# knights-lab/UTree

Measured on NVIDIA B200. Metric: reads/sec (150bp, L2-scale CTR, RC); k-mer lookups/sec in lookups_per_s, higher is better.
Workload: dtype u64

## Files before the change

### utree_b200/csrc/kernels.cu

```cuda
#include <cuda_runtime.h>
#include <stdint.h>
#include <stdio.h>
#include <stdlib.h>
#include <string.h>
#include "utb_internal.h"

#define SUFMASK 0xFFFFFFFFFFull
#define HIT_MISS 0xFFFFFFFFu
#define HIT_NOWIN 0xFFFFFFFEu

#define CK(call)                                                                 \
    do {                                                                         \
        cudaError_t e_ = (call);                                                 \
        if (e_ != cudaSuccess) {                                                 \
            utb_set_error("CUDA error %s at %s:%d (%s)", cudaGetErrorName(e_),   \
                          __FILE__, __LINE__, cudaGetErrorString(e_));           \
            return UTB_ERR_CUDA;                                                 \
        }                                                                        \
    } while (0)

struct DevDB {
    const uint32_t *binix32;
    const uint64_t *binix64;
    const uint8_t *recs;
// ... 354 lines not shown
    if ((uint32_t)p == db.quirk_bin) ++a;
    for (uint64_t i = a + gl; i < b; i += G) {
        const uint64_t word = (p << 40) | load_suffix(db.recs, i * db.sz);
        const uint64_t rc = revcomp_word(word);
        uint32_t *blk = sieve + 2ull * sv_index(db, sv_minimizer(word, rc), sv_block((uint32_t)(word >> 32), (uint32_t)(rc >> 32)));
        const uint2 m = sv_masks((uint32_t)(word >> 32), (uint32_t)word);
        atomicOr(blk + 0, m.x); atomicOr(blk + 1, m.y);
    }
}

#define COUNTER_SLOTS 1024
template <int NSTR, bool TABLE>
__global__ void __launch_bounds__(256, 6)
lookup_kernel(DevDB db, const uint64_t *__restrict__ pk, const uint32_t *__restrict__ bad,
              uint32_t n_pos, const uint32_t *__restrict__ n_groups_dev, uint32_t *__restrict__ hits, unsigned long long *__restrict__ counters) {
    if (n_groups_dev) n_pos = *n_groups_dev * 32u;
    const uint64_t slot = (uint64_t)blockIdx.x * blockDim.x + threadIdx.x;
    const uint32_t pos = (uint32_t)(NSTR == 2 ? slot >> 1 : slot);
    uint64_t w = 0;
    const bool valid = pos < n_pos && window_at(pk, bad, pos, w);
    uint32_t r = HIT_NOWIN, ns = 0;
    if (valid) {
        if (NSTR == 2 && (slot & 1)) w = revcomp_word(w);
        if (TABLE) r = kt_lookup(db, w, &ns);
        else {
            Probe q[1];
            probe_begin(db, w, q[0]);
            probe_run<1>(db, q);
            r = probe_end(db, q[0]);
        }
    }
    if (pos < n_pos) hits[slot] = r;
    const uint32_t nv = __popc(__ballot_sync(0xFFFFFFFFu, valid));
    const uint32_t nh = __popc(__ballot_sync(0xFFFFFFFFu, r < HIT_NOWIN));
    for (int o = 16; o; o >>= 1) ns += __shfl_xor_sync(0xFFFFFFFFu, ns, o);
    if ((threadIdx.x & 31u) == 0) {
        const uint32_t c = blockIdx.x & (COUNTER_SLOTS - 1);
        if (nv) atomicAdd(counters + c, (unsigned long long)nv);
        if (nh) atomicAdd(counters + COUNTER_SLOTS + c, (unsigned long long)nh);
        if (ns) atomicAdd(counters + 3 * COUNTER_SLOTS + c, (unsigned long long)ns);
    }
}

#define Q_CHUNK 128u
#define Q_INVALID 0xFFFFFFFFu
struct WarpQueue {
    uint64_t base;
    uint32_t used;
    bool have;
};
__device__ __forceinline__ void wq_init(WarpQueue &q) { q.base = 0; q.used = Q_CHUNK; q.have = false; }
__device__ __forceinline__ void wq_retire(const WarpQueue &q, uint32_t lane, uint32_t *__restrict__ q_slots) {
    if (q.have) for (uint32_t j = q.used + lane; j < Q_CHUNK; j += 32) q_slots[q.base + j] = Q_INVALID;
}
__device__ __forceinline__ void wq_reserve(WarpQueue &q, uint32_t c, uint32_t lane, uint32_t *__restrict__ q_slots,
                                           unsigned long long *__restrict__ q_count, uint64_t q_cap) {
    if (q.used + c <= Q_CHUNK) return;
    wq_retire(q, lane, q_slots);
    unsigned long long nb = 0;
    if (lane == 0) nb = atomicAdd(q_count, (unsigned long long)Q_CHUNK);
    q.base = __shfl_sync(0xFFFFFFFFu, nb, 0);
    q.used = 0;
    q.have = q.base + Q_CHUNK <= q_cap;
}
struct HitSink {
    uint32_t *hits;
    uint32_t *hitmap;
    const uint32_t *rid, *grp_off;
    uint32_t *cnt;
    uint32_t sh;
};
__device__ __forceinline__ void sink_put(const HitSink &k, uint32_t slot, uint32_t r) {
    if (k.cnt) {
        const uint32_t rd = __ldg(k.rid + (slot >> k.sh));
        k.hits[((uint64_t)__ldg(k.grp_off + rd) << k.sh) + atomicAdd(k.cnt + rd, 1u)] = r;
    } else { k.hits[slot] = r; atomicOr(k.hitmap + (slot >> 5), 1u << (slot & 31u)); }
}
__device__ __noinline__ uint32_t resolve_inline(const DevDB &db, uint64_t w, uint32_t slot, const HitSink &sink) {
    const uint32_t r = kt_lookup(db, w);
    if (r == HIT_MISS) return 0;
    sink_put(sink, slot, r);
    return 1;
}
template <int NSTR>
__device__ __forceinline__ uint32_t emit_survivors(const DevDB &db, WarpQueue &wq, uint32_t lane, bool passF, bool passR, uint64_t w, uint64_t rc,
                                                   uint32_t pos, uint64_t *__restrict__ q_words, uint32_t *__restrict__ q_slots,
                                                   unsigned long long *__restrict__ q_count, uint64_t q_cap, const HitSink &sink) {
    const uint32_t bF = __ballot_sync(0xFFFFFFFFu, passF);
    const uint32_t bR = NSTR == 2 ? __ballot_sync(0xFFFFFFFFu, passR) : 0u;
    const uint32_t cF = __popc(bF), c = cF + __popc(bR);
    uint32_t nh = 0;
    if (!c) return 0;
    wq_reserve(wq, c, lane, q_slots, q_count, q_cap);
    const uint32_t lt = (1u << lane) - 1u;
    if (wq.have) {
        const uint64_t at = wq.base + wq.used;
        if (passF) { const uint64_t i = at + __popc(bF & lt); q_words[i] = w; q_slots[i] = pos * NSTR; }
        if (passR) { const uint64_t i = at + cF + __popc(bR & lt); q_words[i] = rc; q_slots[i] = pos * NSTR + 1u; }
    } else {
        if (passF) nh += resolve_inline(db, w, pos * NSTR, sink);
        if (passR) nh += resolve_inline(db, rc, pos * NSTR + 1u, sink);
    }
    wq.used += c;
    return nh;
}

#define SV_DEAD 0xFFFFFFFFu
struct SvStep { uint32_t wh, wl, rh, rl, h, blk; };
struct SvWords { uint64_t hi, lo, rhi, rlo; uint32_t bh, bl; };
__device__ __forceinline__ void sv_step(const SvWords &g, bool upper, uint32_t r2, uint32_t lane, SvStep &s) {
    const uint32_t b0 = (uint32_t)(g.hi >> 32), b1 = (uint32_t)g.hi, b2 = (uint32_t)(g.lo >> 32), b3 = (uint32_t)g.lo;
    const uint32_t x0 = upper ? b1 : b0, x1 = upper ? b2 : b1, x2 = upper ? b3 : b2;
    s.wh = __funnelshift_l(x1, x0, r2); s.wl = __funnelshift_l(x2, x1, r2);
    const uint32_t a0 = (uint32_t)(g.rlo >> 32), a1 = (uint32_t)g.rlo, a2 = (uint32_t)(g.rhi >> 32), a3 = (uint32_t)g.rhi;
    const uint32_t z0 = upper ? a2 : a3, z1 = upper ? a1 : a2, z2 = upper ? a0 : a1;
    s.rl = __funnelshift_r(z0, z1, r2); s.rh = __funnelshift_r(z1, z2, r2);
    s.h = sv_mhash(s.wh, s.rl);
    s.blk = __funnelshift_r(g.bh, g.bl, lane) == 0u ? sv_block(s.wh, s.rh) : SV_DEAD;
}
template <int D, int SV_U>
__device__ __forceinline__ void sv_shifted(const uint32_t (&x)[SV_U + 1], uint32_t (&y)[SV_U + 1], uint32_t lane) {
    uint32_t rot[SV_U + 1];
#pragma unroll
    for (int u = 0; u <= SV_U; ++u) rot[u] = __shfl_sync(0xFFFFFFFFu, x[u], (lane + D) & 31u);
    const bool same = lane + D < 32u;
#pragma unroll
    for (int u = 0; u < SV_U; ++u) y[u] = same ? rot[u] : rot[u + 1];
    y[SV_U] = rot[SV_U];
}
__device__ __forceinline__ void sv_prefetch(const void *p) { asm volatile("prefetch.global.L1 [%0];" ::"l"(p)); }
template <int NSTR, int SV_U, int SV_MINB>
__global__ void __launch_bounds__(256, SV_MINB)
sieve_kernel(DevDB db, const uint64_t *__restrict__ pk, const uint32_t *__restrict__ bad, const uint64_t *__restrict__ pkr, uint32_t n_pos,
             const uint32_t *__restrict__ n_groups_dev, unsigned long long *__restrict__ counters,
             uint64_t *__restrict__ q_words, uint32_t *__restrict__ q_slots, unsigned long long *__restrict__ q_count,
             uint64_t q_cap, const HitSink sink) {
    if (n_groups_dev) n_pos = *n_groups_dev * 32u;
    const uint32_t lane = threadIdx.x & 31u;
    const bool upper = lane >= 16u;
    const uint32_t r2 = 2u * (lane & 15u);
    const uint32_t n_steps = n_pos >> 5;
    const uint32_t n_warps = gridDim.x * (blockDim.x >> 5), wid = blockIdx.x * (blockDim.x >> 5) + (threadIdx.x >> 5);
    uint32_t per = (n_steps + n_warps - 1) / n_warps;
    per = (per + SV_U - 1) / SV_U * SV_U;
    const uint64_t s0 = (uint64_t)wid * per;
    const uint32_t s1 = s0 + per < n_steps ? (uint32_t)(s0 + per) : n_steps;
    const uint2 *__restrict__ sieve = db.sieve;
    const uint32_t n_lines = db.sv_lines;
    WarpQueue wq;
    wq_init(wq);
    uint32_t nv = 0, nh = 0;
    if (s0 < s1) {
        SvStep st[SV_U + 1];
        SvWords g;
        g.hi = __ldg(pk + s0); g.rhi = __ldg(pkr + s0); g.bh = __ldg(bad + s0);
        g.lo = __ldg(pk + s0 + 1); g.rlo = __ldg(pkr + s0 + 1); g.bl = __ldg(bad + s0 + 1);
        sv_step(g, upper, r2, lane, st[0]);
        for (uint32_t s = (uint32_t)s0; s < s1; s += SV_U) {
            {
                const uint32_t pf = s + 32u < n_steps ? s + 32u : n_steps;
                sv_prefetch(pk + pf); sv_prefetch(pkr + pf); sv_prefetch(bad + pf);
            }
#pragma unroll
            for (int u = 1; u <= SV_U; ++u) {
                g.hi = g.lo; g.rhi = g.rlo; g.bh = g.bl;
                g.lo = __ldg(pk + s + u + 1); g.rlo = __ldg(pkr + s + u + 1); g.bl = __ldg(bad + s + u + 1);
                sv_step(g, upper, r2, lane, st[u]);
            }
            uint32_t x[SV_U + 1], y1[SV_U + 1], y2[SV_U + 1];
#pragma unroll
            for (int u = 0; u <= SV_U; ++u) x[u] = st[u].h;
            sv_shifted<1, SV_U>(x, y1, lane); sv_shifted<2, SV_U>(x, y2, lane);
#pragma unroll
            for (int u = 0; u <= SV_U; ++u) x[u] = __vimin3_u32(x[u], y1[u], y2[u]);
            sv_shifted<3, SV_U>(x, y1, lane); sv_shifted<6, SV_U>(x, y2, lane);
#pragma unroll
            for (int u = 0; u <= SV_U; ++u) x[u] = __vimin3_u32(x[u], y1[u], y2[u]);
            sv_shifted<8, SV_U>(x, y1, lane);
#pragma unroll
            for (int u = 0; u < SV_U; ++u) x[u] = x[u] < y1[u] ? x[u] : y1[u];
            uint2 v[SV_U];
#pragma unroll
            for (int u = 0; u < SV_U; ++u) {
                v[u] = make_uint2(0, 0);
                if (st[u].blk != SV_DEAD) v[u] = __ldg(sieve + ((sv_line(x[u], n_lines) << 4) | st[u].blk));
            }
#pragma unroll
            for (int u = 0; u < SV_U; ++u) {
                const bool live = st[u].blk != SV_DEAD;
                if (__any_sync(0xFFFFFFFFu, live)) {
                    const bool tF = sv_test(v[u], st[u].wh, st[u].wl), tR = NSTR == 2 && sv_test(v[u], st[u].rh, st[u].rl);
                    nh += emit_survivors<NSTR>(db, wq, lane, live & tF, live & tR, ((uint64_t)st[u].wh << 32) | st[u].wl, ((uint64_t)st[u].rh << 32) | st[u].rl,
                                               (s + u) * 32u + lane, q_words, q_slots, q_count, q_cap, sink);
                    nv += live ? NSTR : 0;
                }
            }
            st[0] = st[SV_U];
        }
    }
    wq_retire(wq, lane, q_slots);
    for (int o = 16; o; o >>= 1) { nv += __shfl_xor_sync(0xFFFFFFFFu, nv, o); nh += __shfl_xor_sync(0xFFFFFFFFu, nh, o); }
    if (lane == 0) {
        const uint32_t cs = (blockIdx.x * 8 + (threadIdx.x >> 5)) & (COUNTER_SLOTS - 1);
        if (nv) atomicAdd(counters + cs, (unsigned long long)nv);
        if (nh) atomicAdd(counters + COUNTER_SLOTS + cs, (unsigned long long)nh);
    }
}

template <bool LISTS>
__global__ void __launch_bounds__(256, 6)
queue_lookup_kernel(DevDB db, const uint64_t *__restrict__ q_words, const uint32_t *__restrict__ q_slots,
                    const unsigned long long *__restrict__ q_count, uint64_t q_cap,
                    const HitSink sink, unsigned long long *__restrict__ counters) {
    const uint64_t n = *q_count < q_cap ? *q_count : q_cap;
    const uint64_t stride = (uint64_t)gridDim.x * blockDim.x;
    const uint32_t lane = threadIdx.x & 31u;
    uint32_t nh = 0, nsect = 0;
    for (uint64_t i = (uint64_t)blockIdx.x * blockDim.x + threadIdx.x; i < n; i += stride) {
        const uint32_t slot = q_slots[i];
        uint32_t r = HIT_MISS;
        if (slot != Q_INVALID) {
            uint32_t sc;
            r = kt_lookup(db, q_words[i], &sc);
            nsect += sc;
        }
        const bool hit = r != HIT_MISS;
        nh += hit;
        if (!LISTS) {
            if (hit) { sink.hits[slot] = r; atomicOr(sink.hitmap + (slot >> 5), 1u << (slot & 31u)); }
            continue;
        }
        if (!__any_sync(0xFFFFFFFFu, hit)) continue;
        const uint32_t rd = hit ? __ldg(sink.rid + (slot >> sink.sh)) : 0xFFFFFFFFu;
        const uint32_t peers = __match_any_sync(0xFFFFFFFFu, rd);
        const uint32_t leader = (uint32_t)__ffs(peers) - 1u;
        uint32_t base = 0;
        if (hit && lane == leader) base = atomicAdd(sink.cnt + rd, (uint32_t)__popc(peers));
        base = __shfl_sync(0xFFFFFFFFu, base, leader);
        if (hit) sink.hits[((uint64_t)__ldg(sink.grp_off + rd) << sink.sh) + base + __popc(peers & ((1u << lane) - 1u))] = r;
    }
    for (int o = 16; o; o >>= 1) { nh += __shfl_xor_sync(0xFFFFFFFFu, nh, o); nsect += __shfl_xor_sync(0xFFFFFFFFu, nsect, o); }
    if (lane == 0) {
        const uint32_t c = blockIdx.x & (COUNTER_SLOTS - 1);
        if (nh) atomicAdd(counters + COUNTER_SLOTS + c, (unsigned long long)nh);
        if (nsect) atomicAdd(counters + 3 * COUNTER_SLOTS + c, (unsigned long long)nsect);
    }
}

template <bool TABLE>
__global__ void lookup_words_kernel(DevDB db, const uint64_t *__restrict__ words, uint64_t n, uint32_t *__restrict__ ix) {
    uint64_t i = (uint64_t)blockIdx.x * blockDim.x + threadIdx.x;
    if (i >= n) return;
    if (TABLE) {
        if (db.sieve && !sv_maybe(db, words[i])) { ix[i] = HIT_MISS; return; }
        ix[i] = kt_lookup(db, words[i]);
        return;
    }
    Probe q[1];
    probe_begin(db, words[i], q[0]);
    probe_run<1>(db, q);
    ix[i] = probe_end(db, q[0]);
}


__global__ void expand_windows_kernel(const uint64_t *__restrict__ pk, const uint32_t *__restrict__ bad, uint32_t n_pos,
                                      uint64_t *__restrict__ fwd, uint64_t *__restrict__ rc, uint8_t *__restrict__ valid) {
    uint32_t pos = blockIdx.x * blockDim.x + threadIdx.x;
    if (pos >= n_pos) return;
    uint64_t w;
    bool ok = window_at(pk, bad, pos, w);
    fwd[pos] = ok ? w : 0;
    rc[pos] = ok ? revcomp_word(w) : 0;
    valid[pos] = ok;
}

__device__ __forceinline__ uint32_t cutoff_of(uint32_t x) {
    uint32_t c = x - x / 4u;
    c += ((x >> 1) >= c);
    return c;
}

__device__ __forceinline__ unsigned long long nz_bytes(unsigned long long v) {
    return (((v & 0x7F7F7F7F7F7F7F7Full) + 0x7F7F7F7F7F7F7F7Full) | v) & 0x8080808080808080ull;
}
__device__ __forceinline__ uint32_t scan_token(const char *s1, const char *s2, uint32_t t, char &a, char &b) {
    uint32_t tb = t & ~7u;
    unsigned long long keep = ~0ull << (8u * (t & 7u));
    for (;;) {
        const unsigned long long x1 = *reinterpret_cast<const unsigned long long *>(s1 + tb);
        const unsigned long long x2 = *reinterpret_cast<const unsigned long long *>(s2 + tb);
        const unsigned long long stop = ((nz_bytes(x1) & nz_bytes(x1 ^ 0x3B3B3B3B3B3B3B3Bull)) ^ 0x8080808080808080ull | nz_bytes(x1 ^ x2)) & keep;
        if (stop) {
            const uint32_t k = ((uint32_t)__ffsll((long long)stop) - 1u) >> 3;
            a = (char)(x1 >> (8u * k)); b = (char)(x2 >> (8u * k));
            return tb + k;
        }
        tb += 8u; keep = ~0ull;
    }
}

__device__ void walk_warp(const DevDB &db, const uint32_t *T_lab, const uint32_t *T_cnt,
                          uint32_t uix, uint32_t n, utb_result *out) {
    const uint32_t lane = threadIdx.x & 31u;
    const uint32_t EMPTY = 0xFFFFFFFFu;
    uint32_t cutoff = cutoff_of(n), st = 0, ed = uix, dv = EMPTY, orun = n, sl = 0, ol = 0;
    for (;;) {
        uint32_t run = T_cnt[st], td = dv;
        for (uint32_t z = st + 1; z < ed; ++z) {
            const char *s1 = db.blob + __ldg(db.off + T_lab[z - 1]);
            const char *s2 = db.blob + __ldg(db.off + T_lab[z]);
            if (!s1[dv + (dv == EMPTY)]) {
                run = T_cnt[z]; st = z;
                orun -= T_cnt[z - 1];
                cutoff = cutoff_of(orun);
                continue;
            }
            uint32_t t0 = dv + 1u;
            char a, b;
            for (;;) {
                char ca = s1[t0 + lane], cb = s2[t0 + lane];
                uint32_t m = __ballot_sync(0xFFFFFFFFu, ca == 0 || ca != cb || ca == ';');
                if (m) {
// ... 1249 lines not shown
    db->d.rank = (const uint32_t *)db->rank; db->d.by_rank = (const uint32_t *)db->by_rank;
    db->d.ktab = (const uint64_t *)db->ktab; db->d.sieve = (const uint2 *)db->sieve;
    if (db->l2_window && cudaDeviceSetLimit(cudaLimitPersistingL2CacheSize, db->l2_window_bytes) != cudaSuccess) { cudaGetLastError(); db->l2_window = 0; }
    *out = db;
    return UTB_OK;
}

extern "C" void utb_db_free(utb_db *db) {
    if (!db) return;
    cudaSetDevice(db->device);
    cudaFree(db->binix); cudaFree(db->recs); cudaFree(db->blob); cudaFree(db->ktab); cudaFree(db->sieve);
    cudaFree(db->off); cudaFree(db->rank); cudaFree(db->by_rank);
    free(db);
}
extern "C" uint64_t utb_db_hbm_bytes(const utb_db *db) { return db ? db->hbm_bytes : 0; }
extern "C" int utb_db_lookup_mode(const utb_db *db) { return db ? db->use_table : 0; }
extern "C" int utb_db_device(const utb_db *db) { return db ? db->device : -1; }

struct vote_scratch { VoteLong vl; unsigned n_cta; };
static void vs_free(vote_scratch *vs) {
    cudaFree(vs->vl.hist); cudaFree(vs->vl.tlab); cudaFree(vs->vl.tcnt);
    cudaFree(vs->vl.big_hist); cudaFree(vs->vl.big_tlab); cudaFree(vs->vl.big_tcnt); cudaFree(vs->vl.big_list); cudaFree(vs->vl.big_state); cudaFree(vs->vl.work);
    memset(vs, 0, sizeof *vs);
}
static int vs_alloc(const utb_db *db, size_t max_bytes, vote_scratch *vs) {
    memset(vs, 0, sizeof *vs);
    const size_t nl = db->d.max_ix ? db->d.max_ix : 1;
    vs->n_cta = (unsigned)db->sm_count * VB_PER_SM;
    size_t pool = ((size_t)384 << 20) / (12 * nl);
    if (pool > VBIG_POOL_MAX) pool = VBIG_POOL_MAX;
    if (pool < 1) pool = 1;
    vs->vl.pool = (uint32_t)pool;
    vs->vl.split_slots = (size_t)128 << 10;
    (void)max_bytes;
    const char *e = getenv("UTB_VOTE_SPLIT_SLOTS");
    if (e && atoll(e) > 0) vs->vl.split_slots = (unsigned long long)atoll(e);
    vs->vl.sort_max = VB_SORT_MAX;
    e = getenv("UTB_VOTE_SORT_MAX");
    if (e && atoi(e) >= 0 && (uint32_t)atoi(e) < VB_SORT_MAX) vs->vl.sort_max = (uint32_t)atoi(e);
    cudaError_t err = cudaMalloc(&vs->vl.hist, (size_t)vs->n_cta * nl * 4);
    if (err == cudaSuccess) err = cudaMalloc(&vs->vl.tlab, (size_t)vs->n_cta * nl * 4);
    if (err == cudaSuccess) err = cudaMalloc(&vs->vl.tcnt, (size_t)vs->n_cta * nl * 4);
    if (err == cudaSuccess) err = cudaMalloc(&vs->vl.big_hist, pool * nl * 4);
    if (err == cudaSuccess) err = cudaMalloc(&vs->vl.big_tlab, pool * nl * 4);
    if (err == cudaSuccess) err = cudaMalloc(&vs->vl.big_tcnt, pool * nl * 4);
    if (err == cudaSuccess) err = cudaMalloc(&vs->vl.big_list, pool * 4);
    if (err == cudaSuccess) err = cudaMalloc(&vs->vl.big_state, (1 + 2 * pool) * 4);
    if (err == cudaSuccess) err = cudaMalloc(&vs->vl.work, 4);
    if (err == cudaSuccess) err = cudaMemset(vs->vl.hist, 0, (size_t)vs->n_cta * nl * 4);
    if (err == cudaSuccess) err = cudaMemset(vs->vl.big_hist, 0, pool * nl * 4);
    if (err != cudaSuccess) { vs_free(vs); CK(err); }
    return UTB_OK;
}
static int launch_long_vote(const utb_db *db, const VoteIn &in, utb_result *results, const uint32_t *gen_list, const uint32_t *gen_count,
                            vote_scratch *vs, unsigned long long *counters, cudaStream_t st) {
    CK(cudaMemsetAsync(vs->vl.big_state, 0, (1 + 2 * (size_t)vs->vl.pool) * 4, st));
    CK(cudaMemsetAsync(vs->vl.work, 0, 4, st));
    vote_block_kernel<<<vs->n_cta, VB_THREADS, 0, st>>>(db->d, in, results, gen_list, gen_count, vs->vl, counters);
    vote_big_count_kernel<<<(unsigned)db->sm_count * 4, VB_THREADS, 0, st>>>(db->d, in, vs->vl);
    vote_big_finish_kernel<<<vs->vl.pool < (uint32_t)db->sm_count ? vs->vl.pool : (unsigned)db->sm_count, VB_THREADS, 0, st>>>(db->d, vs->vl, results, counters);
    CK(cudaGetLastError());
    return UTB_OK;
}


struct utb_batch {
    utb_db *db;
    cudaStream_t st;
    cudaEvent_t done, ev[7];
    size_t max_bytes, max_reads;
    uint64_t max_groups;
    char *h_bytes; uint64_t *h_seq_off; uint32_t *h_seq_len; uint32_t *h_grp_off;
    utb_result *h_results; unsigned long long *h_counters;
    uint32_t *h_name_off, *h_name_len; char *h_text; uint32_t *h_text_len; size_t text_cap, h_text_cap;
    uint8_t *d_raw; uint64_t *d_seq_off; uint32_t *d_seq_len; uint32_t *d_grp_off;
    uint64_t *d_pk; uint32_t *d_bad; uint32_t *d_hits; uint64_t *d_pkr;
    utb_result *d_results; uint32_t *d_gen_list; uint32_t *d_gen_count; uint32_t *d_warp_list; uint32_t *d_warp_count;
    uint32_t *d_name_off, *d_name_len, *d_line_len, *d_line_off, *d_scan_sums, *d_text_len; char *d_text;
    int want_text; cudaEvent_t text_len_ready; size_t text_prefetched;
    unsigned long long *d_counters;
    vote_scratch vs;
    uint32_t *d_sel_cnt, *d_sel_off, *d_sel, *d_sel_gap, *d_sel_total, *h_sel_cnt, *h_sel, *h_sel_total; size_t sel_cap;
    uint64_t *d_qwords; uint32_t *d_qslots; unsigned long long *d_qcount; uint64_t q_cap;
    uint32_t *d_hitmap;
    uint32_t *d_rid, *d_hcnt;
    size_t n_reads; uint32_t n_groups; int do_rc; int in_flight; int used_sieve, used_lists;
    uint64_t launches;
    uint32_t *d_nl, *d_blk, *d_frame_err, *h_frame_err; int framed_on_device;
    uint32_t *d_frame_info;
    uint32_t *d_dims, *h_dims; const uint32_t *dims_dev;
    size_t in_bytes;
};

extern "C" uint64_t utb_read_slots(uint32_t len) { return ((uint64_t)len + 1 + 31) / 32; }
extern "C" uint64_t utb_batch_max_slots(const utb_batch *b) { return b->max_groups; }
extern "C" char *utb_batch_bytes(utb_batch *b) { return b->h_bytes; }
extern "C" uint64_t *utb_batch_seq_off(utb_batch *b) { return b->h_seq_off; }
extern "C" uint32_t *utb_batch_seq_len(utb_batch *b) { return b->h_seq_len; }
extern "C" size_t utb_batch_max_bytes(const utb_batch *b) { return b->max_bytes; }
extern "C" size_t utb_batch_max_reads(const utb_batch *b) { return b->max_reads; }

extern "C" void utb_batch_destroy(utb_batch *b) {
    if (!b) return;
    cudaSetDevice(b->db->device);
    if (b->st) cudaStreamSynchronize(b->st);
    cudaFreeHost(b->h_bytes); cudaFreeHost(b->h_seq_off); cudaFreeHost(b->h_seq_len); cudaFreeHost(b->h_grp_off);
    cudaFreeHost(b->h_results); cudaFreeHost(b->h_counters);
    cudaFreeHost(b->h_name_off); cudaFreeHost(b->h_name_len); cudaFreeHost(b->h_text); cudaFreeHost(b->h_text_len);
    cudaFree(b->d_name_off); cudaFree(b->d_name_len); cudaFree(b->d_line_len); cudaFree(b->d_line_off); cudaFree(b->d_scan_sums);
    cudaFree(b->d_text_len); cudaFree(b->d_text);
    if (b->text_len_ready) cudaEventDestroy(b->text_len_ready);
    cudaFree(b->d_raw); cudaFree(b->d_seq_off); cudaFree(b->d_seq_len); cudaFree(b->d_grp_off);
    cudaFree(b->d_pk); cudaFree(b->d_bad); cudaFree(b->d_hits); cudaFree(b->d_results); cudaFree(b->d_pkr);
    cudaFree(b->d_gen_list); cudaFree(b->d_gen_count); cudaFree(b->d_warp_list); cudaFree(b->d_warp_count); cudaFree(b->d_counters);
    vs_free(&b->vs);
    cudaFree(b->d_sel_cnt); cudaFree(b->d_sel_off); cudaFree(b->d_sel); cudaFree(b->d_sel_gap); cudaFree(b->d_sel_total);
    cudaFreeHost(b->h_sel_cnt); cudaFreeHost(b->h_sel); cudaFreeHost(b->h_sel_total);
    cudaFree(b->d_qwords); cudaFree(b->d_qslots); cudaFree(b->d_qcount); cudaFree(b->d_hitmap); cudaFree(b->d_rid); cudaFree(b->d_hcnt);
    cudaFree(b->d_nl); cudaFree(b->d_blk); cudaFree(b->d_frame_err); cudaFreeHost(b->h_frame_err);
    cudaFree(b->d_frame_info); cudaFree(b->d_dims); cudaFreeHost(b->h_dims);
    if (b->done) cudaEventDestroy(b->done);
    for (int i = 0; i < 7; ++i) if (b->ev[i]) cudaEventDestroy(b->ev[i]);
    if (b->st) cudaStreamDestroy(b->st);
    free(b);
}

extern "C" int utb_batch_create(utb_db *db, size_t max_bytes, size_t max_reads, utb_batch **out) {
    if (!db || !out || !max_bytes || !max_reads) { utb_set_error("utb_batch_create: bad argument"); return UTB_ERR_ARG; }
    *out = nullptr;
    if (max_bytes + 32 * max_reads >= ((uint64_t)1 << 32) - 4096) {
        utb_set_error("batch too large: positions must fit 32 bits"); return UTB_ERR_LIMIT;
    }
    CK(cudaSetDevice(db->device));
    utb_batch *b = (utb_batch *)calloc(1, sizeof(utb_batch));
    if (!b) { utb_set_error("out of memory"); return UTB_ERR_NOMEM; }
    b->db = db; b->max_bytes = max_bytes; b->max_reads = max_reads;
    b->max_groups = max_bytes / 32 + max_reads + 1;
    size_t npos = (size_t)b->max_groups * 32;
#define BK(call) do { cudaError_t e_ = (call); if (e_ != cudaSuccess) { utb_set_error("CUDA error %s at %s:%d (%s)", cudaGetErrorName(e_), __FILE__, __LINE__, cudaGetErrorString(e_)); utb_batch_destroy(b); return UTB_ERR_CUDA; } } while (0)
    BK(cudaStreamCreateWithFlags(&b->st, cudaStreamNonBlocking));
    BK(cudaEventCreateWithFlags(&b->done, cudaEventDisableTiming));
    for (int i = 0; i < 7; ++i) BK(cudaEventCreate(&b->ev[i]));
    BK(cudaMallocHost(&b->h_bytes, max_bytes + 64));
    BK(cudaMallocHost(&b->h_seq_off, max_reads * 8));
    BK(cudaMallocHost(&b->h_seq_len, max_reads * 4));
    BK(cudaMallocHost(&b->h_grp_off, (max_reads + 1) * 4));
    BK(cudaMallocHost(&b->h_results, max_reads * sizeof(utb_result)));
    BK(cudaMallocHost(&b->h_counters, 4 * COUNTER_SLOTS * 8));
    BK(cudaMallocHost(&b->h_name_off, (max_reads + 1) * 4));
    BK(cudaMallocHost(&b->h_name_len, (max_reads + 1) * 4));
    BK(cudaMallocHost(&b->h_text_len, 4));
    BK(cudaEventCreateWithFlags(&b->text_len_ready, cudaEventDisableTiming));
    BK(cudaMalloc(&b->d_name_off, (max_reads + 1) * 4));
    BK(cudaMalloc(&b->d_name_len, (max_reads + 1) * 4));
    BK(cudaMalloc(&b->d_line_len, (max_reads + 1) * 4));
    BK(cudaMalloc(&b->d_line_off, (max_reads + 1) * 4));
    BK(cudaMalloc(&b->d_scan_sums, (max_reads / SCAN_TILE + 2) * 4));
    BK(cudaMalloc(&b->d_text_len, 4));
    BK(cudaMalloc(&b->d_dims, 8));
    BK(cudaMallocHost(&b->h_dims, 8));
    BK(cudaMalloc(&b->d_raw, max_bytes + 128));
    BK(cudaMalloc(&b->d_seq_off, max_reads * 8));
    BK(cudaMalloc(&b->d_seq_len, max_reads * 4));
    BK(cudaMalloc(&b->d_grp_off, (max_reads + 1) * 4));
    BK(cudaMalloc(&b->d_pk, (b->max_groups + PK_GUARD + 2) * 8));
    BK(cudaMalloc(&b->d_bad, (b->max_groups + PK_GUARD + 2) * 4));
    BK(cudaMalloc(&b->d_hits, npos * 2 * 4));
    BK(cudaMalloc(&b->d_results, max_reads * sizeof(utb_result)));
    BK(cudaMalloc(&b->d_gen_list, max_reads * 4));
    BK(cudaMalloc(&b->d_gen_count, 4));
    BK(cudaMalloc(&b->d_warp_list, max_reads * 4));
    BK(cudaMalloc(&b->d_warp_count, 4));
    BK(cudaMalloc(&b->d_counters, 4 * COUNTER_SLOTS * 8));
    if (vs_alloc(db, max_bytes, &b->vs)) { utb_batch_destroy(b); return UTB_ERR_CUDA; }
    BK(cudaMemset(b->d_raw, 0, max_bytes + 128));
    if (db->sieve) {
        b->q_cap = npos * 2 / 4 + 4096;
        const char *qc = getenv("UTB_QCAP");
        if (qc && atoll(qc) > 0) b->q_cap = (uint64_t)atoll(qc);
        b->q_cap = (b->q_cap + Q_CHUNK - 1) / Q_CHUNK * Q_CHUNK;
        BK(cudaMalloc(&b->d_qwords, b->q_cap * 8));
        BK(cudaMalloc(&b->d_qslots, b->q_cap * 4));
        BK(cudaMemset(b->d_qslots, 0xFF, b->q_cap * 4));
        BK(cudaMalloc(&b->d_qcount, 8));
        BK(cudaMalloc(&b->d_hitmap, (npos * 2 / 32 + 8) * 4));
        BK(cudaMalloc(&b->d_pkr, (b->max_groups + PK_GUARD + 2) * 8));
        BK(cudaMalloc(&b->d_rid, (b->max_groups + PK_GUARD + 2) * 4));
        BK(cudaMalloc(&b->d_hcnt, (max_reads + 1) * 4));
    }
    if (db->l2_window) {
        cudaStreamAttrValue a;
        memset(&a, 0, sizeof a);
        a.accessPolicyWindow.base_ptr = db->binix;
        a.accessPolicyWindow.num_bytes = db->l2_window_bytes;
        a.accessPolicyWindow.hitRatio = db->l2_hit_ratio;
        a.accessPolicyWindow.hitProp = cudaAccessPropertyPersisting;
        a.accessPolicyWindow.missProp = cudaAccessPropertyStreaming;
        if (cudaStreamSetAttribute(b->st, cudaStreamAttributeAccessPolicyWindow, &a) != cudaSuccess) cudaGetLastError();
    }
#undef BK
    *out = b;
    return UTB_OK;
}

static unsigned gs_grid(const utb_batch *b, uint64_t n, uint32_t per, unsigned waves) {
    const uint64_t need = (n + per - 1) / per, cap = (uint64_t)b->db->sm_count * waves;
    return (unsigned)(need < cap ? (need ? need : 1) : cap);
}

static int launch_stages(utb_batch *b, bool timed) {
    const DevDB &d = b->db->d;
    const uint32_t n_reads = (uint32_t)b->n_reads, n_groups = b->n_groups;
    const uint32_t n_pos = n_groups * 32u;
    const uint32_t nstr = b->do_rc ? 2u : 1u;
    CK(cudaMemsetAsync(b->d_gen_count, 0, 4, b->st));
    CK(cudaMemsetAsync(b->d_counters, 0, 4 * COUNTER_SLOTS * 8, b->st));
    if (timed) CK(cudaEventRecord(b->ev[0], b->st));
    if (n_reads) {
        pack_kernel<<<gs_grid(b, (uint64_t)n_groups + PK_GUARD, 256, 32), 256, 0, b->st>>>(b->d_raw, b->d_seq_off, b->d_seq_len, b->d_grp_off,
                                                                   n_reads, n_groups, b->dims_dev, b->d_pk, b->d_bad, b->d_pkr, b->d_rid);
        b->launches++;
    }
    if (timed) CK(cudaEventRecord(b->ev[1], b->st));
    if (n_pos) {
        const unsigned nb = (unsigned)(((uint64_t)n_pos * nstr + 255) / 256);
        const bool sieve = b->db->sieve && (b->db->sieve_mode == 1 || (b->db->sieve_mode == 2 && b->db->ema_hit_rate < 0.40));
        const unsigned sms = (unsigned)b->db->sm_count;
        b->used_sieve = sieve; b->used_lists = 0;
        if (b->db->use_table && sieve) {
            CK(cudaMemsetAsync(b->d_qcount, 0, 8, b->st));
            HitSink sink;
            sink.hits = b->d_hits; sink.sh = nstr == 2 ? 6u : 5u;
            const bool lists = b->want_text != 3;
            if (lists) { sink.hitmap = nullptr; sink.rid = b->d_rid; sink.grp_off = b->d_grp_off; sink.cnt = b->d_hcnt;
                         CK(cudaMemsetAsync(b->d_hcnt, 0, ((size_t)n_reads + 1) * 4, b->st)); }
            else { sink.hitmap = b->d_hitmap; sink.rid = nullptr; sink.grp_off = nullptr; sink.cnt = nullptr;
                   CK(cudaMemsetAsync(b->d_hitmap, 0, ((size_t)n_pos * nstr / 32 + 4) * 4, b->st)); }
            b->used_lists = lists;
            if (timed) CK(cudaEventRecord(b->ev[4], b->st));
            static const int sv_variant = [] { const char *e = getenv("UTB_SV_VARIANT"); return e ? atoi(e) : 0; }();
#define SV_LAUNCH(U, MINB) do { \
                const unsigned wb = (n_groups + 8u * U - 1) / (8u * U); \
                const unsigned pb = wb < sms * MINB ? (wb ? wb : 1u) : sms * MINB; \
                if (nstr == 2) sieve_kernel<2, U, MINB><<<pb, 256, 0, b->st>>>(d, b->d_pk, b->d_bad, b->d_pkr, n_pos, b->dims_dev ? b->dims_dev + 1 : nullptr, b->d_counters, b->d_qwords, b->d_qslots, b->d_qcount, b->q_cap, sink); \
                else sieve_kernel<1, U, MINB><<<pb, 256, 0, b->st>>>(d, b->d_pk, b->d_bad, b->d_pkr, n_pos, b->dims_dev ? b->dims_dev + 1 : nullptr, b->d_counters, b->d_qwords, b->d_qslots, b->d_qcount, b->q_cap, sink); } while (0)
            switch (sv_variant) {
            case 1: SV_LAUNCH(4, 3); break;
            case 2: SV_LAUNCH(4, 4); break;
            case 3: SV_LAUNCH(2, 6); break;
            case 4: SV_LAUNCH(5, 3); break;
            default: SV_LAUNCH(6, 3); break;
            }
#undef SV_LAUNCH
            if (timed) CK(cudaEventRecord(b->ev[5], b->st));
            if (lists) queue_lookup_kernel<true><<<sms * 6, 256, 0, b->st>>>(d, b->d_qwords, b->d_qslots, b->d_qcount, b->q_cap, sink, b->d_counters);
            else queue_lookup_kernel<false><<<sms * 6, 256, 0, b->st>>>(d, b->d_qwords, b->d_qslots, b->d_qcount, b->q_cap, sink, b->d_counters);
            b->launches++;
        } else if (b->db->use_table) {
            if (nstr == 2) lookup_kernel<2, true><<<nb, 256, 0, b->st>>>(d, b->d_pk, b->d_bad, n_pos, b->dims_dev ? b->dims_dev + 1 : nullptr, b->d_hits, b->d_counters);
            else lookup_kernel<1, true><<<nb, 256, 0, b->st>>>(d, b->d_pk, b->d_bad, n_pos, b->dims_dev ? b->dims_dev + 1 : nullptr, b->d_hits, b->d_counters);
        } else {
            if (nstr == 2) lookup_kernel<2, false><<<nb, 256, 0, b->st>>>(d, b->d_pk, b->d_bad, n_pos, b->dims_dev ? b->dims_dev + 1 : nullptr, b->d_hits, b->d_counters);
            else lookup_kernel<1, false><<<nb, 256, 0, b->st>>>(d, b->d_pk, b->d_bad, n_pos, b->dims_dev ? b->dims_dev + 1 : nullptr, b->d_hits, b->d_counters);
        }
        b->launches++;
    }
    if (timed) CK(cudaEventRecord(b->ev[2], b->st));
    if (n_reads && b->want_text == 3) {
        VoteIn in;
        in.hits = b->d_hits; in.grp_off = b->d_grp_off; in.seq_len = b->d_seq_len; in.off = nullptr; in.nstr = nstr;
        in.hitmap = b->used_sieve ? b->d_hitmap : nullptr;
        const uint32_t nt = (n_reads + SCAN_TILE - 1) / SCAN_TILE;
        shallow_select_kernel<<<gs_grid(b, n_reads, 128, 32), 128, 0, b->st>>>(d, in, b->d_pk, b->d_bad, n_reads, b->dims_dev, b->d_sel_cnt, b->d_sel_gap);
        scan_sums_kernel<<<gs_grid(b, nt, 1, 8), 256, 0, b->st>>>(b->d_sel_cnt, n_reads, b->dims_dev, nt, b->d_scan_sums);
        scan_top_kernel<<<1, 1024, 0, b->st>>>(b->d_scan_sums, nt, b->d_sel_total);
        scan_apply_kernel<<<gs_grid(b, nt, 1, 8), 256, 0, b->st>>>(b->d_sel_cnt, n_reads, b->dims_dev, nt, b->d_scan_sums, b->d_sel_off);
        shallow_compact_kernel<<<gs_grid(b, n_reads, 128, 32), 128, 0, b->st>>>(in, n_reads, b->dims_dev, b->d_sel_cnt, b->d_sel_off, b->d_sel_gap, b->d_sel);
        b->launches += 5;
    } else if (n_reads) {
        VoteIn in;
        in.hits = b->d_hits; in.grp_off = b->d_grp_off; in.seq_len = b->d_seq_len; in.off = nullptr; in.nstr = nstr;
        in.cnt = b->used_lists ? b->d_hcnt : nullptr;
        if (in.cnt) {
            CK(cudaMemsetAsync(b->d_warp_count, 0, 4, b->st));
            vote_thread_kernel<<<gs_grid(b, n_reads, VT_THREADS, 32), VT_THREADS, 0, b->st>>>(
                d, in, n_reads, b->dims_dev, b->d_results, b->d_warp_list, b->d_warp_count, b->d_counters);
            vote_warp_kernel<<<(unsigned)b->db->sm_count * 6, VW_WARPS * 32, 0, b->st>>>(
                d, in, n_reads, b->dims_dev, b->d_warp_list, b->d_warp_count, b->d_results, b->d_gen_list, b->d_gen_count, b->d_counters);
            b->launches++;
        } else
            vote_warp_kernel<<<gs_grid(b, n_reads, VW_WARPS, 32), VW_WARPS * 32, 0, b->st>>>(
                d, in, n_reads, b->dims_dev, nullptr, nullptr, b->d_results, b->d_gen_list, b->d_gen_count, b->d_counters);
        int rv = launch_long_vote(b->db, in, b->d_results, b->d_gen_list, b->d_gen_count, &b->vs, b->d_counters, b->st);
        if (rv) return rv;
        b->launches += 4;
    }
    if (timed) CK(cudaEventRecord(b->ev[3], b->st));
    CK(cudaGetLastError());
    return UTB_OK;
}

static int ensure_text_buffers(utb_batch *b) {
    if (b->d_text) return UTB_OK;
    size_t cap = b->max_bytes + b->max_reads * (b->db->max_label + 48) + 64;
    if (cap >= ((size_t)1 << 32)) { utb_set_error("batch too large for device-side formatting"); return UTB_ERR_LIMIT; }
    const size_t hcap = b->max_bytes / 2 + ((size_t)8 << 20) < cap ? b->max_bytes / 2 + ((size_t)8 << 20) : cap;
    CK(cudaMalloc(&b->d_text, cap));
    CK(cudaMallocHost(&b->h_text, hcap));
    b->text_cap = cap; b->h_text_cap = hcap;
    return UTB_OK;
}
static int grow_text_staging(utb_batch *b, size_t need) {
    if (need <= b->h_text_cap) return UTB_OK;
    CK(cudaStreamSynchronize(b->st));
    cudaFreeHost(b->h_text); b->h_text = nullptr; b->h_text_cap = 0;
    CK(cudaMallocHost(&b->h_text, need));
    b->h_text_cap = need;
    return UTB_OK;
}
extern "C" int utb_batch_prepare(utb_batch *b, int want_text, int chunked);
static int ensure_shallow_buffers(utb_batch *b);

static int submit_impl(utb_batch *b, const char *src, size_t n_bytes, size_t n_reads, int do_rc, int want_text, uint64_t total_groups);
static int finish_submit(utb_batch *b, size_t n_bytes);
extern "C" int utb_batch_submit(utb_batch *b, size_t n_bytes, size_t n_reads, int do_rc) {
    return submit_impl(b, nullptr, n_bytes, n_reads, do_rc, 0, 0);
}
extern "C" int utb_batch_submit_text(utb_batch *b, size_t n_bytes, size_t n_reads, int do_rc) {
// ... 463 lines not shown
```

Measured before the change: 723.3 million.

## Resolve sieve survivors in-kernel via per-warp shared-memory staging with L2 prefetch

Adds a per-warp shared-memory staging buffer in the sieve kernel. Survivors are collected there and resolved inside the same kernel once the buffer is half full, after issuing L2 prefetches for their table sectors. This avoids the global queue round trip for survivors at low hit rates and overlaps table lookups with sieve work. The staged path is enabled only when the EMA hit rate is between 0.5% and 5% or when forced by an environment variable. It adds 24KB of shared memory per block, which may reduce occupancy, and adds warp-divergent drain loops inside the sieve.

```diff
diff --git a/utree_b200/csrc/kernels.cu b/utree_b200/csrc/kernels.cu
--- a/utree_b200/csrc/kernels.cu
+++ b/utree_b200/csrc/kernels.cu
@@ -460,8 +460,59 @@
     sink_put(sink, slot, r);
     return 1;
 }
-template <int NSTR>
-__device__ __forceinline__ uint32_t emit_survivors(const DevDB &db, WarpQueue &wq, uint32_t lane, bool passF, bool passR, uint64_t w, uint64_t rc,
+template <bool LISTS>
+__device__ __forceinline__ uint32_t resolve_survivor(const DevDB &db, bool valid, uint64_t w, uint32_t slot, const HitSink &sink,
+                                                     uint32_t lane, uint32_t &nsect) {
+    uint32_t r = HIT_MISS;
+    if (valid) {
+        uint32_t sc;
+        r = kt_lookup(db, w, &sc);
+        nsect += sc;
+    }
+    const bool hit = r != HIT_MISS;
+    if (!LISTS) {
+        if (hit) { sink.hits[slot] = r; atomicOr(sink.hitmap + (slot >> 5), 1u << (slot & 31u)); }
+        return hit;
+    }
+    if (!__any_sync(0xFFFFFFFFu, hit)) return 0;
+    const uint32_t rd = hit ? __ldg(sink.rid + (slot >> sink.sh)) : 0xFFFFFFFFu;
+    const uint32_t peers = __match_any_sync(0xFFFFFFFFu, rd);
+    const uint32_t leader = (uint32_t)__ffs(peers) - 1u;
+    uint32_t base = 0;
+    if (hit && lane == leader) base = atomicAdd(sink.cnt + rd, (uint32_t)__popc(peers));
+    base = __shfl_sync(0xFFFFFFFFu, base, leader);
+    if (hit) sink.hits[((uint64_t)__ldg(sink.grp_off + rd) << sink.sh) + base + __popc(peers & ((1u << lane) - 1u))] = r;
+    return hit;
+}
+
+#define SV_STAGE 256u
+struct SvStageArea { uint64_t w[SV_STAGE]; uint32_t slot[SV_STAGE]; };
+__shared__ SvStageArea sv_stage[8];
+__device__ __forceinline__ void sv_drain(const DevDB &db, uint32_t n, uint32_t lane, const HitSink &sink, unsigned long long *__restrict__ counters) {
+    const uint64_t *sw = sv_stage[threadIdx.x >> 5].w;
+    const uint32_t *ss = sv_stage[threadIdx.x >> 5].slot;
+    __syncwarp();
+    for (uint32_t i = lane; i < n; i += 32)
+        asm volatile("prefetch.global.L2 [%0];" ::"l"(db.ktab + __umul64hi(mix64(sw[i]), db.kt_sectors) * 4));
+    uint32_t nh = 0, nsect = 0;
+    for (uint32_t b = 0; b < n; b += 32) {
+        const uint32_t i = b + lane;
+        const bool v = i < n;
+        const uint64_t w = v ? sw[i] : 0ull;
+        const uint32_t slot = v ? ss[i] : 0u;
+        nh += sink.cnt ? resolve_survivor<true>(db, v, w, slot, sink, lane, nsect) : resolve_survivor<false>(db, v, w, slot, sink, lane, nsect);
+    }
+    __syncwarp();
+    for (int o = 16; o; o >>= 1) { nh += __shfl_xor_sync(0xFFFFFFFFu, nh, o); nsect += __shfl_xor_sync(0xFFFFFFFFu, nsect, o); }
+    if (lane == 0) {
+        const uint32_t cs = (blockIdx.x * 8 + (threadIdx.x >> 5)) & (COUNTER_SLOTS - 1);
+        if (nh) atomicAdd(counters + COUNTER_SLOTS + cs, (unsigned long long)nh);
+        if (nsect) atomicAdd(counters + 3 * COUNTER_SLOTS + cs, (unsigned long long)nsect);
+    }
+}
+template <int NSTR, bool STAGE>
+__device__ __forceinline__ uint32_t emit_survivors(const DevDB &db, uint32_t &staged, uint32_t stage_cap, WarpQueue &wq, uint32_t lane,
+                                                   bool passF, bool passR, uint64_t w, uint64_t rc,
                                                    uint32_t pos, uint64_t *__restrict__ q_words, uint32_t *__restrict__ q_slots,
                                                    unsigned long long *__restrict__ q_count, uint64_t q_cap, const HitSink &sink) {
     const uint32_t bF = __ballot_sync(0xFFFFFFFFu, passF);
@@ -469,8 +520,16 @@
     const uint32_t cF = __popc(bF), c = cF + __popc(bR);
     uint32_t nh = 0;
     if (!c) return 0;
+    const uint32_t lt = (1u << lane) - 1u;
+    if (STAGE && staged + c <= stage_cap) {
+        uint64_t *sw = sv_stage[threadIdx.x >> 5].w;
+        uint32_t *ss = sv_stage[threadIdx.x >> 5].slot;
+        if (passF) { const uint32_t i = staged + __popc(bF & lt); sw[i] = w; ss[i] = pos * NSTR; }
+        if (passR) { const uint32_t i = staged + cF + __popc(bR & lt); sw[i] = rc; ss[i] = pos * NSTR + 1u; }
+        staged += c;
+        return 0;
+    }
     wq_reserve(wq, c, lane, q_slots, q_count, q_cap);
-    const uint32_t lt = (1u << lane) - 1u;
     if (wq.have) {
         const uint64_t at = wq.base + wq.used;
         if (passF) { const uint64_t i = at + __popc(bF & lt); q_words[i] = w; q_slots[i] = pos * NSTR; }
@@ -507,12 +566,12 @@
     y[SV_U] = rot[SV_U];
 }
 __device__ __forceinline__ void sv_prefetch(const void *p) { asm volatile("prefetch.global.L1 [%0];" ::"l"(p)); }
-template <int NSTR, int SV_U, int SV_MINB>
+template <int NSTR, int SV_U, int SV_MINB, bool STAGE>
 __global__ void __launch_bounds__(256, SV_MINB)
 sieve_kernel(DevDB db, const uint64_t *__restrict__ pk, const uint32_t *__restrict__ bad, const uint64_t *__restrict__ pkr, uint32_t n_pos,
              const uint32_t *__restrict__ n_groups_dev, unsigned long long *__restrict__ counters,
              uint64_t *__restrict__ q_words, uint32_t *__restrict__ q_slots, unsigned long long *__restrict__ q_count,
-             uint64_t q_cap, const HitSink sink) {
+             uint64_t q_cap, const HitSink sink, uint32_t stage_cap, uint32_t stage_drain) {
     if (n_groups_dev) n_pos = *n_groups_dev * 32u;
     const uint32_t lane = threadIdx.x & 31u;
     const bool upper = lane >= 16u;
@@ -527,6 +586,7 @@
     const uint32_t n_lines = db.sv_lines;
     WarpQueue wq;
     wq_init(wq);
+    uint32_t staged = 0;
     uint32_t nv = 0, nh = 0;
     if (s0 < s1) {
         SvStep st[SV_U + 1];
@@ -568,13 +628,15 @@
                 const bool live = st[u].blk != SV_DEAD;
                 if (__any_sync(0xFFFFFFFFu, live)) {
                     const bool tF = sv_test(v[u], st[u].wh, st[u].wl), tR = NSTR == 2 && sv_test(v[u], st[u].rh, st[u].rl);
-                    nh += emit_survivors<NSTR>(db, wq, lane, live & tF, live & tR, ((uint64_t)st[u].wh << 32) | st[u].wl, ((uint64_t)st[u].rh << 32) | st[u].rl,
+                    nh += emit_survivors<NSTR, STAGE>(db, staged, stage_cap, wq, lane, live & tF, live & tR, ((uint64_t)st[u].wh << 32) | st[u].wl, ((uint64_t)st[u].rh << 32) | st[u].rl,
                                                (s + u) * 32u + lane, q_words, q_slots, q_count, q_cap, sink);
                     nv += live ? NSTR : 0;
                 }
             }
             st[0] = st[SV_U];
-        }
+            if (STAGE && staged >= stage_drain) { sv_drain(db, staged, lane, sink, counters); staged = 0; }
+        }
+        if (STAGE && staged) sv_drain(db, staged, lane, sink, counters);
     }
     wq_retire(wq, lane, q_slots);
     for (int o = 16; o; o >>= 1) { nv += __shfl_xor_sync(0xFFFFFFFFu, nv, o); nh += __shfl_xor_sync(0xFFFFFFFFu, nh, o); }
@@ -596,26 +658,8 @@
     uint32_t nh = 0, nsect = 0;
     for (uint64_t i = (uint64_t)blockIdx.x * blockDim.x + threadIdx.x; i < n; i += stride) {
         const uint32_t slot = q_slots[i];
-        uint32_t r = HIT_MISS;
-        if (slot != Q_INVALID) {
-            uint32_t sc;
-            r = kt_lookup(db, q_words[i], &sc);
-            nsect += sc;
-        }
-        const bool hit = r != HIT_MISS;
-        nh += hit;
-        if (!LISTS) {
-            if (hit) { sink.hits[slot] = r; atomicOr(sink.hitmap + (slot >> 5), 1u << (slot & 31u)); }
-            continue;
-        }
-        if (!__any_sync(0xFFFFFFFFu, hit)) continue;
-        const uint32_t rd = hit ? __ldg(sink.rid + (slot >> sink.sh)) : 0xFFFFFFFFu;
-        const uint32_t peers = __match_any_sync(0xFFFFFFFFu, rd);
-        const uint32_t leader = (uint32_t)__ffs(peers) - 1u;
-        uint32_t base = 0;
-        if (hit && lane == leader) base = atomicAdd(sink.cnt + rd, (uint32_t)__popc(peers));
-        base = __shfl_sync(0xFFFFFFFFu, base, leader);
-        if (hit) sink.hits[((uint64_t)__ldg(sink.grp_off + rd) << sink.sh) + base + __popc(peers & ((1u << lane) - 1u))] = r;
+        const bool v = slot != Q_INVALID;
+        nh += resolve_survivor<LISTS>(db, v, v ? q_words[i] : 0ull, slot, sink, lane, nsect);
     }
     for (int o = 16; o; o >>= 1) { nh += __shfl_xor_sync(0xFFFFFFFFu, nh, o); nsect += __shfl_xor_sync(0xFFFFFFFFu, nsect, o); }
     if (lane == 0) {
@@ -2031,6 +2075,7 @@
     vote_scratch vs;
     uint32_t *d_sel_cnt, *d_sel_off, *d_sel, *d_sel_gap, *d_sel_total, *h_sel_cnt, *h_sel, *h_sel_total; size_t sel_cap;
     uint64_t *d_qwords; uint32_t *d_qslots; unsigned long long *d_qcount; uint64_t q_cap;
+    uint32_t stage_cap, stage_drain; int stage_forced;
     uint32_t *d_hitmap;
     uint32_t *d_rid, *d_hcnt;
     size_t n_reads; uint32_t n_groups; int do_rc; int in_flight; int used_sieve, used_lists;
@@ -2128,6 +2173,10 @@
         const char *qc = getenv("UTB_QCAP");
         if (qc && atoll(qc) > 0) b->q_cap = (uint64_t)atoll(qc);
         b->q_cap = (b->q_cap + Q_CHUNK - 1) / Q_CHUNK * Q_CHUNK;
+        b->stage_cap = SV_STAGE;
+        const char *sc = getenv("UTB_SV_STAGE");
+        if (sc && atoi(sc) >= 0) { b->stage_cap = (uint32_t)atoi(sc) < SV_STAGE ? (uint32_t)atoi(sc) : SV_STAGE; b->stage_forced = 1; }
+        b->stage_drain = b->stage_cap > 1 ? b->stage_cap / 2 : 1;
         BK(cudaMalloc(&b->d_qwords, b->q_cap * 8));
         BK(cudaMalloc(&b->d_qslots, b->q_cap * 4));
         BK(cudaMemset(b->d_qslots, 0xFF, b->q_cap * 4));
@@ -2188,11 +2237,14 @@
             b->used_lists = lists;
             if (timed) CK(cudaEventRecord(b->ev[4], b->st));
             static const int sv_variant = [] { const char *e = getenv("UTB_SV_VARIANT"); return e ? atoi(e) : 0; }();
+            const double hr = b->db->ema_hit_rate;
+            const bool stage = b->stage_cap && (b->stage_forced || (hr >= 0.005 && hr <= 0.05));
 #define SV_LAUNCH(U, MINB) do { \
                 const unsigned wb = (n_groups + 8u * U - 1) / (8u * U); \
                 const unsigned pb = wb < sms * MINB ? (wb ? wb : 1u) : sms * MINB; \
-                if (nstr == 2) sieve_kernel<2, U, MINB><<<pb, 256, 0, b->st>>>(d, b->d_pk, b->d_bad, b->d_pkr, n_pos, b->dims_dev ? b->dims_dev + 1 : nullptr, b->d_counters, b->d_qwords, b->d_qslots, b->d_qcount, b->q_cap, sink); \
-                else sieve_kernel<1, U, MINB><<<pb, 256, 0, b->st>>>(d, b->d_pk, b->d_bad, b->d_pkr, n_pos, b->dims_dev ? b->dims_dev + 1 : nullptr, b->d_counters, b->d_qwords, b->d_qslots, b->d_qcount, b->q_cap, sink); } while (0)
+                const auto k = stage ? (nstr == 2 ? sieve_kernel<2, U, MINB, true> : sieve_kernel<1, U, MINB, true>) \
+                                     : (nstr == 2 ? sieve_kernel<2, U, MINB, false> : sieve_kernel<1, U, MINB, false>); \
+                k<<<pb, 256, 0, b->st>>>(d, b->d_pk, b->d_bad, b->d_pkr, n_pos, b->dims_dev ? b->dims_dev + 1 : nullptr, b->d_counters, b->d_qwords, b->d_qslots, b->d_qcount, b->q_cap, sink, b->stage_cap, b->stage_drain); } while (0)
             switch (sv_variant) {
             case 1: SV_LAUNCH(4, 3); break;
             case 2: SV_LAUNCH(4, 4); break;
```

Result: faster. 742.2 million, median of 6 (+2.6%).
